# Anonymousijcai2024ttnet/scale_imagenet

Hardware: AMD Instinct MI355X
Metric: images/sec ImageNet 224x224, TT-small, MI355X; top-1 exact-match (higher is better)
Workload: dtype u16/u32/u64 packed bits (gate path); f32 as prescaled fp16x2 split operands on the 16-bit MFMA (stem, lin1, lin2); 1 GPU; TT_general_imagenet_v2_small forward, batch=256 224x224 per GPU, bit-packed HIP LUT kernels (BASELINE.json configs[1]); batch_per_gpu=256, global_batch=256, batches_in_flight=2, input=float32 NCHW, normalised (the reference's contract), parallelism=batch shard x1

## Files before the change

### scale_imagenet_amd/csrc/gate_fused.hip

```cpp

#include <type_traits>

#include "ttnet_common.h"

namespace ttnet {

namespace {

#ifndef TT_FUSED_SKIP
#define TT_FUSED_SKIP 0
#endif
constexpr int kSkip = TT_FUSED_SKIP;

constexpr int kFT = 1024;
constexpr int kFBuf = 65536;
constexpr int kFMaxScratch = 160 * 1024 - 2 * kFBuf;

template <int W>
using row_t = std::conditional_t<(W > 32), uint64_t, std::conditional_t<(W > 16), uint32_t, uint16_t>>;

template <int HO>
constexpr int fused_round() {
  constexpr int RG = (HO + 3) / 4, a = kFT / (16 * RG), b = kFMaxScratch / (HO * HO * 4);
  return a < b ? (a < 32 ? a : 32) : (b < 32 ? b : 32);
}

struct FusedArgs {
  int n, C, slices, off34, R;
  const void *x;
  const uint8_t *img_c3;
  const uint8_t *img_dw;
  const uint8_t *t_cf;
  void *y;
  uint32_t *idx;
};

__device__ inline void dma_table(uint8_t *dst, const uint8_t *src) {
  if constexpr (kSkip & 1) return;
  const int lane = threadIdx.x & 63, wave = threadIdx.x >> 6;
#pragma unroll
  for (int k = 0; k < kFBuf / 1024 / (kFT / 64); ++k) {
    const int chunk = wave + k * (kFT / 64);
    __builtin_amdgcn_global_load_lds((const __attribute__((address_space(1))) void *)(src + (size_t)chunk * 1024 + lane * 16),
                                     (__attribute__((address_space(3))) void *)(dst + chunk * 1024), 16, 0, 0);
  }
}

__device__ inline void phase_sync() {
  asm volatile("s_waitcnt vmcnt(0)" ::: "memory");
  __syncthreads();
}

typedef const __attribute__((address_space(3))) uint8_t *lds_bytes_t;
__device__ inline uint32_t lds_addr(const void *p) { return (uint32_t)(uintptr_t)(lds_bytes_t)p; }
__device__ inline uint32_t lds_read_u8(uint32_t addr) { return *(lds_bytes_t)(uintptr_t)addr; }
__device__ inline uint32_t lds_read_u32(uint32_t addr) { return *(const __attribute__((address_space(3))) uint32_t *)(uintptr_t)addr; }

__device__ inline uint32_t spread_nibbles(uint32_t x) {
  uint32_t y = (x | (x << 8)) & 0x00FF00FFu;
  return (y | (y << 4)) & 0x0F0F0F0Fu;
}

typedef uint16_t u16x2 __attribute__((ext_vector_type(2)));

template <int WO, int OX0, int OX1>
__device__ inline void dw_lookup_pair(uint32_t pair, uint32_t base, uint32_t &acc) {
  constexpr uint32_t P0 = OX0 & 15, P1 = OX1 & 15;
  const uint32_t adj = __builtin_bit_cast(uint32_t, __builtin_bit_cast(u16x2, pair) - __builtin_bit_cast(u16x2, P0 | (P1 << 16)));
  if constexpr (OX0 < WO) {
    const uint32_t w = lds_read_u32((pair & 0xFFF0u) | base);
    acc |= __builtin_amdgcn_alignbit(w, w, adj) & (0x00010001u << P0);
  }
  if constexpr (OX1 < WO) {
    const uint32_t w = lds_read_u32(((pair >> 16) & 0xFFF0u) | base);
    acc |= __builtin_amdgcn_alignbit(w, w, adj >> 16) & (0x00010001u << P1);
  }
}

template <int WO, int OXB, int OXS>
__device__ inline void dw_eight(uint32_t R0, uint32_t R1, uint32_t R2, uint32_t R3, uint32_t base, uint32_t &acc) {
  if constexpr (OXB >= WO) return;
  static_assert((OXB >> 4) == ((OXB + 7 * OXS) >> 4), "one accumulator per 16 columns");
  constexpr uint32_t M = 0x0F0F0F0Fu;
  const uint32_t t0 = (R0 & M) | ((R1 << 4) & ~M), u0 = (R2 & M) | ((R3 << 4) & ~M);
  dw_lookup_pair<WO, OXB, OXB + 2 * OXS>(__builtin_amdgcn_perm(u0, t0, 0x05010400u), base, acc);
  dw_lookup_pair<WO, OXB + 4 * OXS, OXB + 6 * OXS>(__builtin_amdgcn_perm(u0, t0, 0x07030602u), base, acc);
  if constexpr (OXB + OXS < WO) {
    const uint32_t t1 = ((R0 >> 4) & M) | (R1 & ~M), u1 = ((R2 >> 4) & M) | (R3 & ~M);
    dw_lookup_pair<WO, OXB + OXS, OXB + 3 * OXS>(__builtin_amdgcn_perm(u1, t1, 0x05010400u), base, acc);
    dw_lookup_pair<WO, OXB + 5 * OXS, OXB + 7 * OXS>(__builtin_amdgcn_perm(u1, t1, 0x07030602u), base, acc);
  }
}

template <int W, int WO>
__device__ inline void dw_row_both(const row_t<W> (&r)[4], uint32_t base, uint32_t &accl, uint32_t &acch) {
  accl = 0;
  acch = 0;
  if constexpr (W > 32) {
    uint32_t plo[4], phi[4], qlo[4], qhi[4];
#pragma unroll
    for (int k = 0; k < 4; ++k) {
      qlo[k] = (uint32_t)r[k];
      qhi[k] = (uint32_t)((uint64_t)r[k] >> 32);
      plo[k] = qlo[k] << 2;
      phi[k] = __builtin_amdgcn_alignbit(qhi[k], qlo[k], 30);
    }
    dw_eight<WO, 0, 2>(plo[0], plo[1], plo[2], plo[3], base, accl);
    dw_eight<WO, 16, 2>(phi[0], phi[1], phi[2], phi[3], base, acch);
    dw_eight<WO, 1, 2>(qlo[0], qlo[1], qlo[2], qlo[3], base, accl);
    dw_eight<WO, 17, 2>(qhi[0], qhi[1], qhi[2], qhi[3], base, acch);
  } else {
    uint32_t p[4], q[4];
#pragma unroll
    for (int k = 0; k < 4; ++k) {
      q[k] = (uint32_t)r[k];
      p[k] = q[k] << 2;
    }
    dw_eight<WO, 0, 2>(p[0], p[1], p[2], p[3], base, accl);
    dw_eight<WO, 1, 2>(q[0], q[1], q[2], q[3], base, accl);
    static_assert(WO <= 16, "a 32-bit input row gives at most 16 output columns");
  }
}

__device__ inline uint32_t maj4_bytes(uint32_t v, uint32_t nb) {
  const uint32_t x = v & nb, y = v | nb;
  return (x | (x >> 8) | (y & (y >> 8))) & 0x00FF00FFu;
}

template <int H, int HO, bool LAST>
__global__ __launch_bounds__(kFT) void gate_block_kernel(FusedArgs a) {
  extern __shared__ __align__(16) uint8_t lds[];
  constexpr int W = H, WO = HO, HP = H / 2, WP = W / 2, PIX = HO * WO;
  constexpr int RG = (HO + 3) / 4;
  constexpr int LPR = WO <= 16 ? 16 : 32, RPW = 64 / LPR;
  using TI = row_t<W>;
  using TOut = row_t<WO>;
  uint8_t *const buf0 = lds, *const buf1 = lds + kFBuf;
  uint32_t *const S = (uint32_t *)(lds + 2 * kFBuf);
  if (lds_addr(lds) & (kFBuf - 1)) __builtin_trap();

  const int strands = a.C / 8, P = strands / 2;
  int st, sl;
  {
    const int b = blockIdx.x, x = b & 7, k = b >> 3;
    if (P >= 8 && P % 8 == 0) {
      const int m = P / 8, pair = x + 8 * (k % m), kk = k / m;
      st = 2 * pair + (kk & 1);
      sl = kk >> 1;
    } else if (P == 4 && (a.slices & 1) == 0) {
      st = 2 * (x >> 1) + (k & 1);
      sl = (x & 1) * (a.slices / 2) + (k >> 1);
    } else {
      st = b % strands;
      sl = b / strands;
    }
  }
  const int n0 = (int)((long long)sl * a.n / a.slices), n1 = (int)((long long)(sl + 1) * a.n / a.slices);
  if (n0 >= n1) return;
  const int q = st >> 1, half = st & 1;
  const int tid0 = threadIdx.x, lane = tid0 & 63;
  const DwLaneConst lk = dw_lane_const(lane);
  auto opaque_tid = [&]() {
    int t = tid0;
    asm volatile("" : "+v"(t));
    return t;
  };
  const TI *const x = (const TI *)a.x;

  const uint8_t *const src_c3 = a.img_c3 + (size_t)st * kFBuf;
  const uint8_t *const src_dw0 = a.img_dw + (size_t)(2 * st) * kFBuf, *const src_dw1 = src_dw0 + kFBuf;
  const uint8_t *const src_cf0 = LAST ? nullptr : a.t_cf + (size_t)(2 * st) * kFBuf, *const src_cf1 = LAST ? nullptr : src_cf0 + kFBuf;

  constexpr int RMAX = fused_round<HO>();
  constexpr int TA = (RMAX * HP + kFT / 16 - 1) / (kFT / 16);
  static_assert(RMAX * RG * 16 <= kFT, "one depthwise task per thread");
  TI ra[TA][2];
  TI rb0[4], rb1[4];
  const int R = a.R;

  auto load_a = [&](int i0, int rn) {
    const int tid = opaque_tid();
    const int c = tid & 15, g = tid >> 4;
#pragma unroll
    for (int p = 0; p < TA; ++p) {
      const int gt = p * (kFT / 16) + g;
      const bool ok = gt < rn * HP;
      const int im = ok ? gt / HP : 0, py = ok ? gt - (gt / HP) * HP : 0;
      const TI *src = x + ((size_t)(n0 + i0 + im) * a.C + 16 * q + c) * H + 2 * py;
      ra[p][0] = ok ? src[0] : (TI)0;
      ra[p][1] = ok ? src[1] : (TI)0;
    }
  };
  auto load_b = [&](int i0, int rn, int sub, TI (&rb)[4]) {
    const int tid = opaque_tid();
    const int c4 = tid & 3, r = (tid >> 2) & 3, gi = tid >> 4;
    const int im = gi / RG, rg = gi - im * RG;
    const int oy = 4 * rg + r;
    const bool ok = im < rn && oy < HO;
    const TI *src = x + ((size_t)(n0 + i0 + (ok ? im : 0)) * a.C + 8 * st + 4 * sub + c4) * H;
#pragma unroll
    for (int kh = 0; kh < 4; ++kh) {
      const int iy = 2 * oy - 2 + kh;
      rb[kh] = (ok && iy >= 0 && iy < H) ? src[iy] : (TI)0;
    }
  };

  auto phase_a = [&](int rn, const uint8_t *tab) {
    if constexpr (kSkip & 2) return;
    const int tid = opaque_tid();
    for (int t = tid; t < rn * (HO + WO - 1); t += kFT) {
      const int im = t / (HO + WO - 1), e = t - im * (HO + WO - 1);
      const int edge = a.off34 ? 0 : HO - 1;
      const int pix = e < WO ? edge * WO + e : (e - WO + (a.off34 ? 1 : 0)) * WO + edge;
      *(uint16_t *)((uint8_t *)(S + im * PIX + pix) + 2) = 0;
    }
    const int g = tid >> 4, j = tid & 15;
    const uint32_t tb = lds_addr(tab);
    constexpr int CHUNKS = W > 32 ? 2 : 1, TPB = 2 / CHUNKS;
    static_assert(TA % TPB == 0, "phase A walks whole batches");
#pragma unroll
    for (int bt = 0; bt < TA / TPB; ++bt) {
      uint32_t d[4];
#pragma unroll
      for (int u = 0; u < 2; ++u) {
        const int p = bt * TPB + (CHUNKS == 2 ? 0 : u), k = CHUNKS == 2 ? u : 0;
        d[2 * u] = (uint32_t)((uint64_t)ra[p][0] >> (32 * k));
        d[2 * u + 1] = (uint32_t)((uint64_t)ra[p][1] >> (32 * k));
      }
      transpose16_multi<4>(d, lk);
      uint32_t v3[2], v4[2];
#pragma unroll
      for (int u = 0; u < 2; ++u) {
        const uint32_t t0 = d[2 * u], t1 = d[2 * u + 1];
        const uint32_t e00 = lds_read_u8((t0 & 0xFFFFu) | tb), e01 = lds_read_u8(__builtin_amdgcn_alignbit(tb >> 16, t0, 16));
        const uint32_t e10 = lds_read_u8((t1 & 0xFFFFu) | tb), e11 = lds_read_u8(__builtin_amdgcn_alignbit(tb >> 16, t1, 16));
        v3[u] = e00 | (e10 << 8) | (e01 << 16) | (e11 << 24);
        v4[u] = __builtin_amdgcn_perm(t1, t0, half ? 0x07030501u : 0x06020400u);
      }
      uint32_t n3[2], n4[2];
#pragma unroll
      for (int u = 0; u < 2; ++u) {
        n3[u] = lane_xor16<1>(v3[u]);
        n4[u] = lane_xor16<1>(v4[u]);
      }
#pragma unroll
      for (int u = 0; u < 2; ++u) {
        const int p = bt * TPB + (CHUNKS == 2 ? 0 : u), k = CHUNKS == 2 ? u : 0;
        const int gt = p * (kFT / 16) + g;
        const bool ok = gt < rn * HP;
        const int im = ok ? gt / HP : 0, py = ok ? gt - (gt / HP) * HP : 0;
        const uint32_t m3 = maj4_bytes(v3[u], n3[u]), m4 = maj4_bytes(v4[u], n4[u]);
        const uint32_t sh = (uint32_t)(j & 1) * 16u;
        const uint32_t t = ((m3 >> sh) & 0xFFu) | (((m4 >> sh) & 0xFFu) << 8);
        const uint32_t dlt = ((t >> 4) ^ t) & 0x00F0u;
        const uint32_t v = t ^ dlt ^ (dlt << 4);
        const int px = 16 * k + 8 * (j & 1) + (j >> 1);
        if (ok && px < WP) {
          const int pix = (py + a.off34) * WO + px + a.off34;
          *(uint16_t *)((uint8_t *)(S + im * PIX + pix) + 2) = (uint16_t)v;
        }
      }
      __builtin_amdgcn_sched_barrier(0);
    }
  };

  uint32_t bacc[2][2];
  auto phase_b_lookup = [&](const uint8_t *tab, int sub, const TI (&rb)[4]) {
    if constexpr (kSkip & 4) return;
    const int tid = opaque_tid();
    dw_row_both<W, WO>(rb, lds_addr(tab) | (uint32_t)(tid & 3) * 4u, bacc[sub][0], bacc[sub][1]);
  };
  auto phase_b_store = [&](int rn) {
    if constexpr (kSkip & 4) return;
    const int tid = opaque_tid();
    const int j = tid & 15, gi = tid >> 4;
    const int im = gi / RG, rg = gi - im * RG;
    constexpr int NT = WO > 16 ? 4 : 2;
    uint32_t t[NT];
    if constexpr (WO > 16) {
      t[0] = bacc[0][0]; t[1] = bacc[1][0]; t[2] = bacc[0][1]; t[3] = bacc[1][1];
    } else {
      t[0] = bacc[0][0]; t[1] = bacc[1][0];
    }
    transpose16_multi<NT>(t, lk);
    uint8_t *dst = (uint8_t *)(S + im * PIX + 4 * rg * WO + j);
    auto put = [&](uint32_t w0, uint32_t w1, int col0) {
      if (im < rn && col0 + j < WO) {
        const uint32_t lo = __builtin_amdgcn_perm(w1, w0, 0x05010400u), hi = __builtin_amdgcn_perm(w1, w0, 0x07030602u);
        if (4 * rg + 0 < HO) *(uint16_t *)(dst + (0 * WO + col0) * 4) = (uint16_t)lo;
        if (4 * rg + 1 < HO) *(uint16_t *)(dst + (1 * WO + col0) * 4) = (uint16_t)(lo >> 16);
        if (4 * rg + 2 < HO) *(uint16_t *)(dst + (2 * WO + col0) * 4) = (uint16_t)hi;
        if (4 * rg + 3 < HO) *(uint16_t *)(dst + (3 * WO + col0) * 4) = (uint16_t)(hi >> 16);
      }
    };
    put(spread_nibbles(t[0] & 0xFFFFu) | (spread_nibbles(t[0] >> 16) << 4), spread_nibbles(t[1] & 0xFFFFu) | (spread_nibbles(t[1] >> 16) << 4), 0);
    if constexpr (WO > 16)
      put(spread_nibbles(t[2] & 0xFFFFu) | (spread_nibbles(t[2] >> 16) << 4), spread_nibbles(t[3] & 0xFFFFu) | (spread_nibbles(t[3] >> 16) << 4), 16);
  };

  auto phase_c = [&](int i0, int rn, const uint8_t *tab, int kgrp) {
    if constexpr (kSkip & 8) return;
    const int tid = opaque_tid();
    const int lane = tid & 63, wave = __builtin_amdgcn_readfirstlane(tid >> 6);
    const int sub = lane / LPR, ox = lane % LPR;
    TOut *const y = (TOut *)a.y;
    constexpr int CH2 = (HO + 2 * RPW - 1) / (2 * RPW);
    constexpr int U = 2, NW = kFT / 64;
    const uint32_t sel = kgrp ? 0x05040301u : 0x05040200u;
    const uint32_t tbh = lds_addr(tab) >> 16;
    if (kgrp == 0 && a.idx)
      for (int t = tid; t < rn * PIX; t += kFT) a.idx[((size_t)(n0 + i0 + t / PIX) * strands + st) * PIX + (t % PIX)] = S[t];
    for (int wt0 = wave; wt0 < rn * CH2; wt0 += U * NW) {
      uint32_t w[U], d0[U], d1[U];
      int im[U], oy[U];
#pragma unroll
      for (int u = 0; u < U; ++u) {
        const int wt = wt0 + u * NW;
        im[u] = wt / CH2;
        oy[u] = (wt - im[u] * CH2) * 2 * RPW + sub;
        const bool live = wt < rn * CH2 && ox < WO;
        d0[u] = live && oy[u] < HO ? S[im[u] * PIX + oy[u] * WO + ox] : 0u;
        d1[u] = live && oy[u] + RPW < HO ? S[im[u] * PIX + (oy[u] + RPW) * WO + ox] : 0u;
      }
#pragma unroll
      for (int u = 0; u < U; ++u)
        w[u] = ox < WO ? lds_read_u8(__builtin_amdgcn_perm(tbh, d0[u], sel)) | (lds_read_u8(__builtin_amdgcn_perm(tbh, d1[u], sel)) << 8)
                       : 0u;
      transpose16_multi<U>(w, lk);
#pragma unroll
      for (int u = 0; u < U; ++u) {
        const uint32_t piece = w[u] & 0xFFFFu;
        uint32_t rowbits = piece;
        if constexpr (LPR == 32) rowbits |= (uint32_t)__shfl_xor((int)piece, 16) << 16;
        const int row = oy[u] + ((lane >> 3) & 1) * RPW;
        if (wt0 + u * NW < rn * CH2 && (lane & (LPR - 1)) < 16 && row < HO)
          y[((uint32_t)(n0 + i0 + im[u]) * (uint32_t)(2 * a.C) + 16 * st + 8 * kgrp + (lane & 7)) * HO + row] = (TOut)rowbits;
      }
    }
  };

  auto phase_out = [&](int i0, int rn) {
    const int tid = opaque_tid();
    for (int t = tid; t < rn * PIX; t += kFT)
      a.idx[((size_t)(n0 + i0 + t / PIX) * strands + st) * PIX + (t % PIX)] = S[t];
  };

  const int total = n1 - n0;
  int cur = 0;
  load_a(0, min(R, total));
  dma_table(buf0, src_c3);
  for (int i0 = 0; i0 < total; i0 += R) {
    const int rn = min(R, total - i0);
    const bool more = i0 + R < total;
    uint8_t *tb = cur ? buf1 : buf0, *nb = cur ? buf0 : buf1;
    phase_sync();
    load_b(i0, rn, 0, rb0);
    dma_table(nb, src_dw0);
    phase_a(rn, tb);
    cur ^= 1; tb = cur ? buf1 : buf0; nb = cur ? buf0 : buf1;
    phase_sync();
    load_b(i0, rn, 1, rb1);
    dma_table(nb, src_dw1);
    phase_b_lookup(tb, 0, rb0);
    cur ^= 1; tb = cur ? buf1 : buf0; nb = cur ? buf0 : buf1;
    phase_sync();
    if constexpr (LAST) {
      if (more) {
        load_a(i0 + R, min(R, total - i0 - R));
        dma_table(nb, src_c3);
      }
      phase_b_lookup(tb, 1, rb1);
      phase_b_store(rn);
      cur ^= 1;
      phase_sync();
      phase_out(i0, rn);
    } else {
      dma_table(nb, src_cf0);
      phase_b_lookup(tb, 1, rb1);
      phase_b_store(rn);
      cur ^= 1; tb = cur ? buf1 : buf0; nb = cur ? buf0 : buf1;
      phase_sync();
      dma_table(nb, src_cf1);
      phase_c(i0, rn, tb, 0);
      cur ^= 1; tb = cur ? buf1 : buf0; nb = cur ? buf0 : buf1;
      phase_sync();
      if (more) {
        load_a(i0 + R, min(R, total - i0 - R));
        dma_table(nb, src_c3);
      }
      phase_c(i0, rn, tb, 1);
      cur ^= 1;
    }
  }
}

__global__ void c3_image_kernel(const uint16_t *__restrict__ t_c3, uint8_t *__restrict__ img, int strands) {
  const size_t t = (size_t)blockIdx.x * blockDim.x + threadIdx.x;
  if (t >= (size_t)strands * 65536) return;
  const int st = (int)(t >> 16);
  const uint32_t idx = (uint32_t)(t & 0xFFFF);
  img[t] = (uint8_t)(t_c3[(size_t)(st >> 1) * 65536 + idx] >> (8 * (st & 1)));
}
__global__ void dw_image_kernel(const uint32_t *__restrict__ t1, const uint32_t *__restrict__ t2, uint32_t *__restrict__ img, int C) {
  const size_t t = (size_t)blockIdx.x * blockDim.x + threadIdx.x;
  if (t >= (size_t)C * 2048 * 2) return;
  const int ch = (int)(t & 3), d = (int)((t >> 2) & 4095), ss = (int)(t >> 14);
  const int channel = 4 * ss + ch, row = d >> 1, up = d & 1;
  const size_t src = ((size_t)(channel >> 4) * 2048 + row) * 16 + (channel & 15);
  const uint32_t h1 = (t1[src] >> (16 * up)) & 0xFFFFu, h2 = (t2[src] >> (16 * up)) & 0xFFFFu;
  img[t] = up ? (h1 << 16) | h2 : h1 | (h2 << 16);
}

__global__ void branch_rows_kernel(const uint32_t *__restrict__ idx, uint64_t *__restrict__ rows, int n, int C, int HO, int br) {
  const size_t t = (size_t)blockIdx.x * blockDim.x + threadIdx.x;
  if (t >= (size_t)n * C * HO) return;
  const int oy = (int)(t % HO), c = (int)((t / HO) % C), im = (int)(t / ((size_t)HO * C));
  const int st = c >> 3, k = c & 7;
  const int shift = 8 * ((br >> 1) * 2 + (k >> 2)) + 4 * (br & 1) + (k & 3);
  const uint32_t *src = idx + ((size_t)im * (C / 8) + st) * HO * HO + (size_t)oy * HO;
  uint64_t r = 0;
  for (int ox = 0; ox < HO; ++ox) r |= (uint64_t)((src[ox] >> shift) & 1u) << ox;
  rows[t] = r;
}
template <typename T>
__global__ void widen_rows_kernel(const T *__restrict__ src, uint64_t *__restrict__ dst, size_t count) {
  const size_t t = (size_t)blockIdx.x * blockDim.x + threadIdx.x;
  if (t < count) dst[t] = (uint64_t)src[t];
}
template <typename T>
__global__ void narrow_rows_kernel(const uint64_t *__restrict__ src, T *__restrict__ dst, size_t count) {
  const size_t t = (size_t)blockIdx.x * blockDim.x + threadIdx.x;
  if (t < count) dst[t] = (T)src[t];
}

template <int H, int HO, bool LAST>
int launch_block_t(const FusedBlockArgs &f, hipStream_t s) {
  auto k = gate_block_kernel<H, HO, LAST>;
  constexpr int PIX = HO * HO;
  const int strands = f.C / 8;
  int R = fused_round<HO>();
  const int slices = fused_block_slices(f.C, f.n);
  R = std::max(1, std::min(R, (f.n + slices - 1) / slices));
  const size_t lds = (size_t)2 * kFBuf + (size_t)R * PIX * 4;
  TT_TRY(ensure_dynamic_lds((const void *)k, kMaxLds));
  FusedArgs a{};
  a.n = f.n; a.C = f.C; a.slices = slices; a.off34 = f.off34; a.R = R;
  a.x = f.x; a.img_c3 = (const uint8_t *)f.img_c3; a.img_dw = (const uint8_t *)f.img_dw; a.t_cf = f.t_cf; a.y = f.y; a.idx = f.idx;
  hipLaunchKernelGGL(k, dim3(strands * slices), dim3(kFT), lds, s, a);
  TT_HIP(hipGetLastError());
  return TTNET_OK;
}

}

int row_bytes(int W) { return W > 32 ? 8 : (W > 16 ? 4 : 2); }

int fused_block_slices(int C, int n) {
  const int strands = C / 8;
  int slices = std::max(1, std::min(n, 256 / strands));
  if (strands == 8 && slices > 1 && (slices & 1)) slices -= 1;
  return slices;
}

bool fused_block_supported(int C, int H, int Ho, int stride, int pad, int kh, int kw) {
  if (stride != 2 || pad != 2 || kh != 4 || kw != 4 || C % 16) return false;
  return (H == 56 && Ho == 29) || (H == 29 && Ho == 15) || (H == 15 && Ho == 8) || (H == 8 && Ho == 5);
}

int launch_gate_block(const FusedBlockArgs &f, hipStream_t s) {
  if (f.last && !f.idx) {
    set_error("gate_block: a last block needs its branch-dword buffer");
    return TTNET_E_INVALID;
  }
#define TT_FUSED_CASE(h, ho)                                                         \
  if (f.H == h && f.Ho == ho) return f.last ? launch_block_t<h, ho, true>(f, s) : launch_block_t<h, ho, false>(f, s)
  if (f.H == 56 && f.Ho == 29 && !f.last) return launch_block_t<56, 29, false>(f, s);
  TT_FUSED_CASE(29, 15);
  TT_FUSED_CASE(15, 8);
  TT_FUSED_CASE(8, 5);
#undef TT_FUSED_CASE
  set_error("gate_block: no fused kernel for %dx%d -> %dx%d", f.H, f.H, f.Ho, f.Ho);
  return TTNET_E_UNSUPPORTED;
}

int launch_fused_images(const void *t_dw1, const void *t_dw2, const void *t_c3, int C, void *img_dw, void *img_c3, hipStream_t s) {
  {
    const size_t t = (size_t)(C / 8) * 65536;
    hipLaunchKernelGGL(c3_image_kernel, dim3((unsigned)((t + 255) / 256)), dim3(256), 0, s, (const uint16_t *)t_c3, (uint8_t *)img_c3,
                       C / 8);
  }
  {
    const size_t t = (size_t)C * 2048 * 2;
    hipLaunchKernelGGL(dw_image_kernel, dim3((unsigned)((t + 255) / 256)), dim3(256), 0, s, (const uint32_t *)t_dw1,
                       (const uint32_t *)t_dw2, (uint32_t *)img_dw, C);
  }
  TT_HIP(hipGetLastError());
  return TTNET_OK;
}

int launch_branch_rows(const uint32_t *idx, uint64_t *rows, int n, int C, int Ho, int branch, hipStream_t s) {
  const size_t t = (size_t)n * C * Ho;
  hipLaunchKernelGGL(branch_rows_kernel, dim3((unsigned)((t + 255) / 256)), dim3(256), 0, s, idx, rows, n, C, Ho, branch);
  TT_HIP(hipGetLastError());
  return TTNET_OK;
}

int launch_widen_rows(const void *src, uint64_t *dst, size_t count, int W, hipStream_t s) {
  const unsigned g = (unsigned)((count + 255) / 256);
  if (W > 32) hipLaunchKernelGGL(widen_rows_kernel<uint64_t>, dim3(g), dim3(256), 0, s, (const uint64_t *)src, dst, count);
  else if (W > 16) hipLaunchKernelGGL(widen_rows_kernel<uint32_t>, dim3(g), dim3(256), 0, s, (const uint32_t *)src, dst, count);
  else hipLaunchKernelGGL(widen_rows_kernel<uint16_t>, dim3(g), dim3(256), 0, s, (const uint16_t *)src, dst, count);
  TT_HIP(hipGetLastError());
  return TTNET_OK;
}

int launch_narrow_rows(const uint64_t *src, void *dst, size_t count, int W, hipStream_t s) {
  const unsigned g = (unsigned)((count + 255) / 256);
  if (W > 32) hipLaunchKernelGGL(narrow_rows_kernel<uint64_t>, dim3(g), dim3(256), 0, s, src, (uint64_t *)dst, count);
  else if (W > 16) hipLaunchKernelGGL(narrow_rows_kernel<uint32_t>, dim3(g), dim3(256), 0, s, src, (uint32_t *)dst, count);
  else hipLaunchKernelGGL(narrow_rows_kernel<uint16_t>, dim3(g), dim3(256), 0, s, src, (uint16_t *)dst, count);
  TT_HIP(hipGetLastError());
  return TTNET_OK;
}

}
```

Baseline: 2.091 million images/s.

## Use buffer loads/stores with OOB clamping and reciprocal division in fused gate kernel

Global input loads, output row stores and index-tap stores in the fused gate block kernel now go through AMD buffer resource descriptors. Per-lane bound checks are replaced by out-of-range offsets that the hardware returns as zero or drops, and 64-bit address math becomes 32-bit offsets. Integer divisions by non-power-of-two constants are replaced with compile-time-verified 24-bit multiply-shift reciprocals. LDS writes and reads now use precomputed per-lane byte addresses. The aim is fewer VALU instructions for addressing and predication, at the cost of a new channel-count limit and reliance on buffer OOB semantics.

```diff
diff --git a/scale_imagenet_amd/csrc/gate_fused.hip b/scale_imagenet_amd/csrc/gate_fused.hip
--- a/scale_imagenet_amd/csrc/gate_fused.hip
+++ b/scale_imagenet_amd/csrc/gate_fused.hip
@@ -60,6 +60,50 @@
   uint32_t y = (x | (x << 8)) & 0x00FF00FFu;
   return (y | (y << 4)) & 0x0F0F0F0Fu;
 }
+
+constexpr uint32_t kOob = 0x7FFF0000u;
+constexpr int kRsrcFlags = 0x00020000;
+typedef uint32_t u32x2 __attribute__((ext_vector_type(2)));
+
+template <typename T>
+__device__ inline T buf_load(__amdgpu_buffer_rsrc_t rs, uint32_t voff, uint32_t soff) {
+  if constexpr (sizeof(T) == 8) return (T)__builtin_bit_cast(uint64_t, __builtin_amdgcn_raw_buffer_load_b64(rs, (int)voff, (int)soff, 0));
+  else if constexpr (sizeof(T) == 4) return (T)__builtin_amdgcn_raw_buffer_load_b32(rs, (int)voff, (int)soff, 0);
+  else return (T)__builtin_amdgcn_raw_buffer_load_b16(rs, (int)voff, (int)soff, 0);
+}
+template <typename T>
+__device__ inline void buf_store(T v, __amdgpu_buffer_rsrc_t rs, uint32_t voff, uint32_t soff) {
+  static_assert(sizeof(T) == 4 || sizeof(T) == 2, "output rows and branch dwords");
+  if constexpr (sizeof(T) == 4) __builtin_amdgcn_raw_buffer_store_b32((uint32_t)v, rs, (int)voff, (int)soff, 0);
+  else __builtin_amdgcn_raw_buffer_store_b16((uint16_t)v, rs, (int)voff, (int)soff, 0);
+}
+
+template <int D, int MAXV>
+struct SmallDiv {
+  static constexpr bool exact(int s) {
+    const uint64_t m = (((uint64_t)1 << s) + D - 1) / D;
+    if (m >= (1u << 24) || (uint64_t)MAXV * m >= ((uint64_t)1 << 32)) return false;
+    for (uint64_t v = 0; v <= (uint64_t)MAXV; ++v)
+      if (((v * m) >> s) != v / D) return false;
+    return true;
+  }
+  static constexpr int pick() {
+    for (int s = 8; s < 32; ++s)
+      if (exact(s)) return s;
+    return -1;
+  }
+  static constexpr int S = pick();
+  static_assert(S > 0 && MAXV < (1 << 24), "no 24-bit reciprocal divides this range exactly");
+  static constexpr uint32_t M = (uint32_t)((((uint64_t)1 << S) + D - 1) / D);
+  template <int ADD = 0>
+  __device__ static inline uint32_t div(uint32_t v) {
+    if constexpr ((D & (D - 1)) == 0) return (v + ADD) / D;
+    else return (__umul24(v, M) + (uint32_t)ADD * M) >> S;
+  }
+};
+
+typedef __attribute__((address_space(3))) uint16_t *lds_u16_t;
+__device__ inline void lds_write_u16(uint32_t addr, uint32_t v) { *(lds_u16_t)(uintptr_t)addr = (uint16_t)v; }
 
 typedef uint16_t u16x2 __attribute__((ext_vector_type(2)));
 
@@ -165,7 +209,6 @@
     asm volatile("" : "+v"(t));
     return t;
   };
-  const TI *const x = (const TI *)a.x;
 
   const uint8_t *const src_c3 = a.img_c3 + (size_t)st * kFBuf;
   const uint8_t *const src_dw0 = a.img_dw + (size_t)(2 * st) * kFBuf, *const src_dw1 = src_dw0 + kFBuf;
@@ -174,47 +217,62 @@
   constexpr int RMAX = fused_round<HO>();
   constexpr int TA = (RMAX * HP + kFT / 16 - 1) / (kFT / 16);
   static_assert(RMAX * RG * 16 <= kFT, "one depthwise task per thread");
+  static_assert((RG & (RG - 1)) == 0, "gi / RG is a shift");
   TI ra[TA][2];
   TI rb0[4], rb1[4];
   const int R = a.R;
 
+  constexpr uint32_t SZ = sizeof(TI), CHB = H * SZ;
+  const uint32_t img_in = (uint32_t)a.C * CHB;
+  auto in_rows = [&](int i0, int rn) {
+    return __builtin_amdgcn_make_buffer_rsrc((void *)((const uint8_t *)a.x + (size_t)(n0 + i0) * img_in), 0, (int)(rn * img_in), kRsrcFlags);
+  };
+  using DivHP = SmallDiv<HP, TA * (kFT / 16) - 1>;
+
   auto load_a = [&](int i0, int rn) {
     const int tid = opaque_tid();
-    const int c = tid & 15, g = tid >> 4;
-#pragma unroll
-    for (int p = 0; p < TA; ++p) {
-      const int gt = p * (kFT / 16) + g;
-      const bool ok = gt < rn * HP;
-      const int im = ok ? gt / HP : 0, py = ok ? gt - (gt / HP) * HP : 0;
-      const TI *src = x + ((size_t)(n0 + i0 + im) * a.C + 16 * q + c) * H + 2 * py;
-      ra[p][0] = ok ? src[0] : (TI)0;
-      ra[p][1] = ok ? src[1] : (TI)0;
-    }
+    const uint32_t c = tid & 15, g = tid >> 4;
+    const __amdgpu_buffer_rsrc_t rs = in_rows(i0, rn);
+    const uint32_t soff = (uint32_t)(16 * q) * CHB;
+    const uint32_t lane_off = c * CHB + g * (2 * SZ), per_im = img_in - HP * 2 * SZ;
+    static_for<0, TA>([&](auto pc) {
+      constexpr int p = decltype(pc)::value;
+      const uint32_t off = __umul24(DivHP::template div<p * (kFT / 16)>(g), per_im) + lane_off;
+      ra[p][0] = buf_load<TI>(rs, off + p * (kFT / 16) * 2 * SZ, soff);
+      ra[p][1] = buf_load<TI>(rs, off + p * (kFT / 16) * 2 * SZ + SZ, soff);
+    });
   };
   auto load_b = [&](int i0, int rn, int sub, TI (&rb)[4]) {
     const int tid = opaque_tid();
-    const int c4 = tid & 3, r = (tid >> 2) & 3, gi = tid >> 4;
-    const int im = gi / RG, rg = gi - im * RG;
-    const int oy = 4 * rg + r;
-    const bool ok = im < rn && oy < HO;
-    const TI *src = x + ((size_t)(n0 + i0 + (ok ? im : 0)) * a.C + 8 * st + 4 * sub + c4) * H;
-#pragma unroll
-    for (int kh = 0; kh < 4; ++kh) {
-      const int iy = 2 * oy - 2 + kh;
-      rb[kh] = (ok && iy >= 0 && iy < H) ? src[iy] : (TI)0;
-    }
+    const uint32_t c4 = tid & 3, r = (tid >> 2) & 3, gi = tid >> 4;
+    const uint32_t im = gi / RG, oy = 4 * (gi % RG) + r;
+    const __amdgpu_buffer_rsrc_t rs = in_rows(i0, rn);
+    const uint32_t soff = (uint32_t)(8 * st + 4 * sub) * CHB;
+    static_assert(2 * HO >= H && 2 * HO - 3 <= H - 1, "the window rows of oy < HO, and only those, can lie inside the picture");
+    const uint32_t mid = __umul24(im, img_in) + c4 * CHB + oy * (2 * SZ);
+    const uint32_t up = oy - 1 < (uint32_t)(HO - 1) ? mid - 2 * SZ : kOob;
+    const uint32_t dn0 = 2 * oy < (uint32_t)H ? mid : kOob, dn1 = 2 * oy + 1 < (uint32_t)H ? mid : kOob;
+    rb[0] = buf_load<TI>(rs, up, soff);
+    rb[1] = buf_load<TI>(rs, up + SZ, soff);
+    rb[2] = buf_load<TI>(rs, dn0, soff);
+    rb[3] = buf_load<TI>(rs, dn1 + SZ, soff);
   };
 
   auto phase_a = [&](int rn, const uint8_t *tab) {
     if constexpr (kSkip & 2) return;
     const int tid = opaque_tid();
-    for (int t = tid; t < rn * (HO + WO - 1); t += kFT) {
-      const int im = t / (HO + WO - 1), e = t - im * (HO + WO - 1);
-      const int edge = a.off34 ? 0 : HO - 1;
-      const int pix = e < WO ? edge * WO + e : (e - WO + (a.off34 ? 1 : 0)) * WO + edge;
-      *(uint16_t *)((uint8_t *)(S + im * PIX + pix) + 2) = 0;
-    }
-    const int g = tid >> 4, j = tid & 15;
+    constexpr int BORDER = HO + WO - 1;
+    static_assert(RMAX * BORDER <= kFT, "one border element per thread");
+    const uint32_t s_bytes = lds_addr(S) + 2;
+    if (tid < rn * BORDER) {
+      const uint32_t im = SmallDiv<BORDER, RMAX * BORDER - 1>::div((uint32_t)tid), e = (uint32_t)tid - __umul24(im, BORDER);
+      const uint32_t edge = a.off34 ? 0 : HO - 1;
+      const uint32_t pix = e < (uint32_t)WO ? edge * WO + e : (e - WO + (a.off34 ? 1 : 0)) * WO + edge;
+      lds_write_u16(s_bytes + 4 * (__umul24(im, PIX) + pix), 0);
+    }
+    const uint32_t g = tid >> 4, j = tid & 15;
+    const uint32_t lane_dst = s_bytes + 4 * ((uint32_t)a.off34 * (WO + 1) + 8 * (j & 1) + (j >> 1)) + g * (4 * WO);
+    const int tasks = rn * HP;
     const uint32_t tb = lds_addr(tab);
     constexpr int CHUNKS = W > 32 ? 2 : 1, TPB = 2 / CHUNKS;
     static_assert(TA % TPB == 0, "phase A walks whole batches");
@@ -246,18 +304,15 @@
 #pragma unroll
       for (int u = 0; u < 2; ++u) {
         const int p = bt * TPB + (CHUNKS == 2 ? 0 : u), k = CHUNKS == 2 ? u : 0;
-        const int gt = p * (kFT / 16) + g;
-        const bool ok = gt < rn * HP;
-        const int im = ok ? gt / HP : 0, py = ok ? gt - (gt / HP) * HP : 0;
         const uint32_t m3 = maj4_bytes(v3[u], n3[u]), m4 = maj4_bytes(v4[u], n4[u]);
         const uint32_t sh = (uint32_t)(j & 1) * 16u;
         const uint32_t t = ((m3 >> sh) & 0xFFu) | (((m4 >> sh) & 0xFFu) << 8);
         const uint32_t dlt = ((t >> 4) ^ t) & 0x00F0u;
         const uint32_t v = t ^ dlt ^ (dlt << 4);
-        const int px = 16 * k + 8 * (j & 1) + (j >> 1);
-        if (ok && px < WP) {
-          const int pix = (py + a.off34) * WO + px + a.off34;
-          *(uint16_t *)((uint8_t *)(S + im * PIX + pix) + 2) = (uint16_t)v;
+        const uint32_t px = 16 * k + 8 * (j & 1) + (j >> 1);
+        if ((int)g < tasks - p * (kFT / 16) && px < (uint32_t)WP) {
+          const uint32_t im = DivHP::div(g + p * (kFT / 16));
+          lds_write_u16(__umul24(im, 4 * (PIX - HP * WO)) + lane_dst + (p * (kFT / 16) * 4 * WO + 16 * k * 4), v);
         }
       }
       __builtin_amdgcn_sched_barrier(0);
@@ -273,8 +328,9 @@
   auto phase_b_store = [&](int rn) {
     if constexpr (kSkip & 4) return;
     const int tid = opaque_tid();
-    const int j = tid & 15, gi = tid >> 4;
-    const int im = gi / RG, rg = gi - im * RG;
+    const int j = tid & 15;
+    const uint32_t gi = tid >> 4;
+    const int im = (int)(gi / RG), rg = (int)(gi % RG);
     constexpr int NT = WO > 16 ? 4 : 2;
     uint32_t t[NT];
     if constexpr (WO > 16) {
@@ -283,7 +339,7 @@
       t[0] = bacc[0][0]; t[1] = bacc[1][0];
     }
     transpose16_multi<NT>(t, lk);
-    uint8_t *dst = (uint8_t *)(S + im * PIX + 4 * rg * WO + j);
+    uint8_t *dst = (uint8_t *)(S + __umul24((uint32_t)im, PIX) + 4 * rg * WO + j);
     auto put = [&](uint32_t w0, uint32_t w1, int col0) {
       if (im < rn && col0 + j < WO) {
         const uint32_t lo = __builtin_amdgcn_perm(w1, w0, 0x05010400u), hi = __builtin_amdgcn_perm(w1, w0, 0x07030602u);
@@ -298,52 +354,69 @@
       put(spread_nibbles(t[2] & 0xFFFFu) | (spread_nibbles(t[2] >> 16) << 4), spread_nibbles(t[3] & 0xFFFFu) | (spread_nibbles(t[3] >> 16) << 4), 16);
   };
 
+  auto tap_dwords = [&](int i0, int rn, int tid) {
+    const uint32_t img_idx = (uint32_t)strands * (PIX * 4);
+    const __amdgpu_buffer_rsrc_t ri =
+        __builtin_amdgcn_make_buffer_rsrc((void *)((uint8_t *)a.idx + (size_t)(n0 + i0) * img_idx), 0, (int)(rn * img_idx), kRsrcFlags);
+    const uint32_t s0 = lds_addr(S);
+    for (int t = tid; t < rn * PIX; t += kFT) {
+      const uint32_t im = SmallDiv<PIX, RMAX * PIX - 1>::div((uint32_t)t);
+      buf_store<uint32_t>(lds_read_u32(s0 + 4 * t), ri, __umul24(im, img_idx - PIX * 4) + 4 * t, (uint32_t)st * (PIX * 4));
+    }
+  };
+
   auto phase_c = [&](int i0, int rn, const uint8_t *tab, int kgrp) {
     if constexpr (kSkip & 8) return;
     const int tid = opaque_tid();
-    const int lane = tid & 63, wave = __builtin_amdgcn_readfirstlane(tid >> 6);
-    const int sub = lane / LPR, ox = lane % LPR;
-    TOut *const y = (TOut *)a.y;
+    const uint32_t lane = tid & 63;
+    const int wave = __builtin_amdgcn_readfirstlane(tid >> 6);
+    const uint32_t sub = lane / LPR, ox = lane % LPR;
     constexpr int CH2 = (HO + 2 * RPW - 1) / (2 * RPW);
     constexpr int U = 2, NW = kFT / 64;
+    constexpr int TAIL = HO - (CH2 - 1) * 2 * RPW;
+    constexpr uint32_t SZO = sizeof(TOut);
     const uint32_t sel = kgrp ? 0x05040301u : 0x05040200u;
     const uint32_t tbh = lds_addr(tab) >> 16;
-    if (kgrp == 0 && a.idx)
-      for (int t = tid; t < rn * PIX; t += kFT) a.idx[((size_t)(n0 + i0 + t / PIX) * strands + st) * PIX + (t % PIX)] = S[t];
+    if (kgrp == 0 && a.idx) tap_dwords(i0, rn, tid);
+    const uint32_t img_out = (uint32_t)(2 * a.C) * (HO * SZO);
+    const __amdgpu_buffer_rsrc_t ry =
+        __builtin_amdgcn_make_buffer_rsrc((void *)((uint8_t *)a.y + (size_t)(n0 + i0) * img_out), 0, (int)(rn * img_out), kRsrcFlags);
+    const uint32_t y_strand = (uint32_t)(16 * st + 8 * kgrp) * (HO * SZO);
+    const uint32_t lrow = sub + ((lane >> 3) & 1) * RPW;
+    const uint32_t y_lane = (lane & (LPR - 1)) < 16 ? (lane & 7) * (HO * SZO) + lrow * SZO : kOob;
+    const uint32_t y_tail = lrow < (uint32_t)TAIL ? y_lane : kOob;
+    const uint32_t s_lane = lds_addr(S) + 4 * (sub * WO + ox);
+    const bool col = ox < (uint32_t)WO, tail0 = col && sub < (uint32_t)TAIL, tail1 = col && sub + RPW < (uint32_t)TAIL;
     for (int wt0 = wave; wt0 < rn * CH2; wt0 += U * NW) {
       uint32_t w[U], d0[U], d1[U];
-      int im[U], oy[U];
 #pragma unroll
       for (int u = 0; u < U; ++u) {
         const int wt = wt0 + u * NW;
-        im[u] = wt / CH2;
-        oy[u] = (wt - im[u] * CH2) * 2 * RPW + sub;
-        const bool live = wt < rn * CH2 && ox < WO;
-        d0[u] = live && oy[u] < HO ? S[im[u] * PIX + oy[u] * WO + ox] : 0u;
-        d1[u] = live && oy[u] + RPW < HO ? S[im[u] * PIX + (oy[u] + RPW) * WO + ox] : 0u;
+        const int im = wt / CH2, ch = wt - im * CH2;
+        const bool live = wt < rn * CH2, tail = ch == CH2 - 1;
+        const uint32_t sa = s_lane + (uint32_t)(4 * (im * PIX + ch * 2 * RPW * WO));
+        d0[u] = live && (tail ? tail0 : col) ? lds_read_u32(sa) : 0u;
+        d1[u] = live && (tail ? tail1 : col) ? lds_read_u32(sa + RPW * WO * 4) : 0u;
       }
 #pragma unroll
       for (int u = 0; u < U; ++u)
-        w[u] = ox < WO ? lds_read_u8(__builtin_amdgcn_perm(tbh, d0[u], sel)) | (lds_read_u8(__builtin_amdgcn_perm(tbh, d1[u], sel)) << 8)
-                       : 0u;
+        w[u] = col ? lds_read_u8(__builtin_amdgcn_perm(tbh, d0[u], sel)) | (lds_read_u8(__builtin_amdgcn_perm(tbh, d1[u], sel)) << 8)
+                   : 0u;
       transpose16_multi<U>(w, lk);
 #pragma unroll
       for (int u = 0; u < U; ++u) {
         const uint32_t piece = w[u] & 0xFFFFu;
         uint32_t rowbits = piece;
         if constexpr (LPR == 32) rowbits |= (uint32_t)__shfl_xor((int)piece, 16) << 16;
-        const int row = oy[u] + ((lane >> 3) & 1) * RPW;
-        if (wt0 + u * NW < rn * CH2 && (lane & (LPR - 1)) < 16 && row < HO)
-          y[((uint32_t)(n0 + i0 + im[u]) * (uint32_t)(2 * a.C) + 16 * st + 8 * kgrp + (lane & 7)) * HO + row] = (TOut)rowbits;
-      }
-    }
-  };
-
-  auto phase_out = [&](int i0, int rn) {
-    const int tid = opaque_tid();
-    for (int t = tid; t < rn * PIX; t += kFT)
-      a.idx[((size_t)(n0 + i0 + t / PIX) * strands + st) * PIX + (t % PIX)] = S[t];
-  };
+        const int wt = wt0 + u * NW;
+        const int im = wt / CH2, ch = wt - im * CH2;
+        if (wt < rn * CH2)
+          buf_store<TOut>((TOut)rowbits, ry, ch == CH2 - 1 ? y_tail : y_lane, (uint32_t)im * img_out + y_strand + (uint32_t)(ch * 2 * RPW) * SZO);
+      }
+    }
+  };
+
+  auto phase_out = [&](int i0, int rn) { tap_dwords(i0, rn, opaque_tid()); };
 
   const int total = n1 - n0;
   int cur = 0;
@@ -435,6 +508,10 @@
 
 template <int H, int HO, bool LAST>
 int launch_block_t(const FusedBlockArgs &f, hipStream_t s) {
+  if (f.C > 16384) {
+    set_error("gate_block: %d channels are more than the fused kernel addresses", f.C);
+    return TTNET_E_UNSUPPORTED;
+  }
   auto k = gate_block_kernel<H, HO, LAST>;
   constexpr int PIX = HO * HO;
   const int strands = f.C / 8;
```

Measured after the change: 2.130 million images/s (median of 5 runs). Within noise of the previous version (+1.8%).
